# DaehwanKimLab/centrifuge

Hardware: AMD Instinct MI355X
Metric: classified reads/sec (whole node) on 100bp synthetic reads vs p_compressed; HBM GB/s achieved (higher is better)
Workload: dtype u64

## Files before the change

centrifuge_amd/csrc/cf_device.hip:

```cpp
#include <hip/hip_runtime.h>
#include <sched.h>
#include <dlfcn.h>

#include <algorithm>
#include <cmath>
#include <chrono>
#include <cstdio>
#include <cstdlib>
#include <cstring>
#include <memory>
#include <mutex>
#include <stdexcept>
#include <string>
#include <vector>

#include "../../include/centrifuge_amd.h"
#include "cf_index.hpp"
#include "cf_kernels.hpp"
#include "cf_scan.hpp"
#include "cf_textio.hpp"
#include "cf_restore.hpp"
#include "cf_plan.hpp"
#include "cf_knobs.hpp"

// ... 16 lines not shown
        if (e_ != hipSuccess)                                                                     \
            throw HipError(std::string(#expr) + ": " + hipGetErrorString(e_));                    \
    } while (0)

static thread_local uint64_t *g_dryBytes = nullptr;
template <typename T>
struct DevBuf {
    T *p = nullptr;
    size_t n = 0;
    DevBuf() = default;
    DevBuf(const DevBuf &) = delete;
    DevBuf &operator=(const DevBuf &) = delete;
    ~DevBuf() { release(); }
    void release() { if (p) (void)hipFree(p); p = nullptr; n = 0; }
    void alloc(size_t count) {
        release();
        if (count == 0) count = 1;
        if (g_dryBytes) { *g_dryBytes += count * sizeof(T); n = count; return; }
        HIP_OK(hipMalloc(reinterpret_cast<void **>(&p), count * sizeof(T)));
        n = count;
    }
    void ensure(size_t count) { if (count > n) alloc(count + count / 8); }
    void upload(const std::vector<T> &v) {
        alloc(v.size());
        if (!v.empty()) HIP_OK(hipMemcpy(p, v.data(), v.size() * sizeof(T), hipMemcpyHostToDevice));
    }
    size_t bytes() const { return n * sizeof(T); }
};

template <int G>
__global__ void __launch_bounds__(256) k_search(DIndex ix, DParams pr, DBatch b) { search_body<G>(ix, pr, b); }

__global__ void __launch_bounds__(256) k_rlen(const uint64_t *off, uint32_t *rlen, uint32_t nReads) { rlen_body(off, rlen, nReads, cf_global_thread()); }
__global__ void __launch_bounds__(256) k_convert(DConvert c) { convert_body(c, cf_global_thread()); }
__global__ void __launch_bounds__(256) k_dense_unpack(DUnpack u) { dense_unpack_body(u, (uint64_t)blockIdx.x * blockDim.x + threadIdx.x); }
__global__ void __launch_bounds__(256) k_pack(DBatch b, uint8_t *recs, uint32_t W) { pack_body(b, recs, W, cf_global_thread()); }

template <int G, int W, bool COUNT>
__global__ void __launch_bounds__(256) __attribute__((amdgpu_waves_per_eu(COUNT ? 1 : W == 4 ? 6 : W == 6 ? 5 : 4, 8))) k_search2(DIndex ix, DParams pr, DBatch b) {
    __shared__ __attribute__((aligned(16))) uint8_t lds[(256 / G) * rec_lds_stride(W) + 256 * 4 * RankTab<G>::WORDS + (256 / G) * 16 * kLazyHits];
    search2_body<G, W, COUNT>(ix, pr, b, lds);
}

template <int W, bool COUNT, int LZ = 0, bool MULTI = false>
__global__ void __launch_bounds__(256) __attribute__((amdgpu_waves_per_eu((W == 4 && LZ == 1) ? 7 : (W == 4 && MULTI) ? 6 : (W == 6 && MULTI) ? 5 : 1, 8))) k_search2_l1(DIndex ix, DParams pr, DBatch b) {
    __shared__ __attribute__((aligned(16))) uint8_t lds[256 * rec_lds_stride(W) + 256 * 16 * (LZ ? LZ : (int)lazy_hits(1, W))];
    search2_body<1, W, COUNT, true, LZ, MULTI>(ix, pr, b, lds);
}
__global__ void __launch_bounds__(256) k_pair_planes(DIndex ix, uint8_t *planes2, uint64_t nGroups) {
    pair_planes_body(ix, planes2, (uint64_t)blockIdx.x * blockDim.x + threadIdx.x, nGroups);
}
__global__ void __launch_bounds__(256) k_occ_planes(DIndex ix, uint8_t *planes, uint64_t nSides) {
    occ_planes_body(ix, planes, (uint64_t)blockIdx.x * blockDim.x + threadIdx.x, nSides);
}
__global__ void __launch_bounds__(256) k_repeat_probe(DIndex ix, uint32_t nSamples, uint32_t depth, uint32_t *hits) {
    const uint32_t i = cf_global_thread();
    bool yes = false;
    if (i < nSamples && ix.len > 2) {
        uint64_t x = 0x9e3779b97f4a7c15ull * (i + 1);
        x ^= x >> 29; x *= 0xbf58476d1ce4e5b9ull; x ^= x >> 32;
        yes = repeat_probe_body(ix, x % (ix.len - 1), depth);
    }
    const uint64_t m = cf_ballot(yes);
    if (m && cf_lane() == (uint32_t)cf_ctz64(m)) (void)cf_atomic_add(hits, (uint32_t)cf_popc64(m));
}

__global__ void __launch_bounds__(256) k_post_fast(DIndex ix, DParams pr, DBatch b) {
    const uint32_t q = cf_global_thread();
    const bool d = q < b.nQueries ? post_fast_body(ix, pr, b, q) : false;
    if (q < b.nQueries && b.postDeferred) b.postDeferred[q] = d ? 1 : 0;
    defer_push(b.slowPost, &b.st->nSlowPost, d, q);
}
template <bool EARLY>
__global__ void __launch_bounds__(256) k_score_fast(DIndex ix, DParams pr, DBatch b) {
    const uint32_t q = cf_global_thread();
    const bool d = q < b.nQueries ? score_fast_body<EARLY>(ix, pr, b, q) : false;
    defer_push(b.slowScore, &b.st->nSlowScore, d, q);
}
__global__ void __launch_bounds__(256) k_list_all(uint32_t *list, uint32_t *counter, uint32_t n) {
    const uint32_t q = cf_global_thread();
    if (q < n) list[q] = q;
    if (q == 0) *counter = n;
}
__global__ void __launch_bounds__(64) __attribute__((amdgpu_waves_per_eu(3, 8))) k_post(DIndex ix, DParams pr, DBatch b, uint32_t capHits) {
    extern __shared__ __attribute__((aligned(16))) uint8_t ldsPost[];
    HitP *scratch = capHits ? reinterpret_cast<HitP *>(ldsPost) + (size_t)cf_local_thread() * capHits : nullptr;
    const uint32_t n = b.st->nSlowPost;
    for (uint32_t i = cf_global_thread(); i < n; i += cf_global_threads()) post_body(ix, pr, b, b.slowPost[i], scratch, capHits);
}
__global__ void __launch_bounds__(64) k_postfix_only(DIndex ix, DParams pr, DBatch b) {
    const uint32_t i = cf_global_thread();
    if (i < b.st->nItems / 2) post_fix(ix, pr, b, b.items[i]);
}
__global__ void k_window(DBatch b, uint32_t qLo, bool keepSlow) { if (cf_global_thread() == 0) row_window_body(b, qLo, keepSlow); }
__global__ void __launch_bounds__(256) k_emit(DParams pr, DBatch b) {
    const uint32_t q = cf_global_thread();
    if (q < b.nQueries) emit_body(pr, b, q);
}
template <int G, bool COUNT>
__global__ void __launch_bounds__(256) k_walk2(DIndex ix, DBatch b) { walk2_body<G, COUNT>(ix, b); }
template <int MODE>
__global__ void __launch_bounds__(256) k_walk_table(DIndex ix, DBatch b) { walk2_body<2, false, MODE>(ix, b); }
template <typename T>
__global__ void __launch_bounds__(256) k_stop_samples(DIndex ix, T *stopVal, uint64_t *stopBits, uint64_t nSamples) {
    for (uint64_t i = (uint64_t)blockIdx.x * blockDim.x + threadIdx.x; i < nSamples; i += (uint64_t)gridDim.x * blockDim.x) {
        const uint64_t pos = trio_at(ix.saPos, i << ix.offRate);
        stopVal[pos] = static_cast<const T *>(ix.offs)[i];
        cf_atomic_or64(&stopBits[pos >> 6], 1ull << (pos & 63));
    }
}
template <typename T>
__global__ void __launch_bounds__(256) k_stop_bounds(DIndex ix, T *stopVal, uint64_t *stopBits) {
    for (uint64_t j = (uint64_t)blockIdx.x * blockDim.x + threadIdx.x; j < ix.nBound; j += (uint64_t)gridDim.x * blockDim.x) {
        const uint64_t pos = trio_at(ix.saPos, ix.boundRow[j]);
        stopVal[pos] = (T)ix.boundRef[j];
        cf_atomic_or64(&stopBits[pos >> 6], 1ull << (pos & 63));
    }
}
template <typename T>
__global__ void k_stop_end(DIndex ix, T *stopVal, uint64_t *stopBits) {
    const uint64_t pos = trio_at(ix.saPos, ix.zOff);
    stopVal[pos] = 0;
    cf_atomic_or64(&stopBits[pos >> 6], 1ull << (pos & 63));
}
template <typename T>
__global__ void __launch_bounds__(256) k_table_by_position(DIndex ix, const T *stopVal, const uint64_t *stopBits, T *table, uint64_t nRows, uint32_t *walkMax) {
    uint32_t gap = 0;
    for (uint64_t row = (uint64_t)blockIdx.x * blockDim.x + threadIdx.x; row < nRows; row += (uint64_t)gridDim.x * blockDim.x) {
        const uint64_t pos = trio_at(ix.saPos, row);
        uint64_t w = pos >> 6;
        uint64_t m = stopBits[w] & (~0ull >> (63 - (pos & 63)));
        while (m == 0 && w > 0) m = stopBits[--w];
        const uint64_t pred = m ? (w << 6) + 63 - (uint64_t)__builtin_clzll(m) : 0;
        table[row] = stopVal[pred];
        const uint32_t g = (uint32_t)(pos - pred);
        gap = g > gap ? g : gap;
    }
    for (int d = 32; d > 0; d >>= 1) { const uint32_t o = __shfl_xor(gap, d, 64); gap = o > gap ? o : gap; }
    if ((threadIdx.x & 63) == 0 && gap) atomicMax(walkMax, gap);
}
template <typename T>
__global__ void __launch_bounds__(256) k_table_spot_check(DIndex ix, const T *table, uint64_t nRows, uint32_t nCheck, uint32_t *bad) {
    const uint32_t i = blockIdx.x * blockDim.x + threadIdx.x;
    if (i >= nCheck) return;
    const uint64_t row = i < 64 ? (i < 32 ? (uint64_t)i : nRows - 1 - (i - 32)) % nRows : (0x9e3779b97f4a7c15ull * (i + 1)) % nRows;
    uint32_t steps = 0;
    const uint32_t want = resolve_plain_row(ix, row, steps);
    if ((uint32_t)table[row] != (sizeof(T) == 2 ? (want & 0xffffu) : want)) atomicAdd(bad, 1u);
}

template <bool COUNT>
__global__ void __launch_bounds__(256) k_walk3(DIndex ix, DBatch b) {
    for (uint64_t i = (uint64_t)blockIdx.x * blockDim.x + threadIdx.x; i < b.st->rowHi - b.st->rowLo; i += (uint64_t)gridDim.x * blockDim.x)
        walk3_body<COUNT>(ix, b, i);
}
template <bool PLANES>
__global__ void __launch_bounds__(256) k_wide_ftab(DIndex ix, uint32_t wideChars, uint64_t *table) {
    __builtin_assume(PLANES ? ix.planes != nullptr : ix.planes == nullptr);
    for (uint64_t t = (uint64_t)blockIdx.x * blockDim.x + threadIdx.x; t < (1ull << (2 * wideChars)); t += (uint64_t)gridDim.x * blockDim.x)
        wide_ftab_body(ix, wideChars, table, t);
}

__global__ void __launch_bounds__(64) k_resolve_slow(DIndex ix, DParams pr, DBatch b) {
    const uint32_t n = b.st->nSlowScore;
    for (uint32_t i = cf_global_thread(); i < n; i += cf_global_threads()) resolve_query_body(ix, pr, b, b.slowScore[i]);
}
__global__ void __launch_bounds__(64) k_score(DIndex ix, DParams pr, DBatch b, uint32_t capRows, uint32_t sparse, uint32_t rowsMin, uint32_t rowsMax) {
    extern __shared__ __attribute__((aligned(16))) uint8_t ldsScore[];
    const uint32_t n = b.st->nSlowScore;
    if (cf_local_thread() % sparse) return;
    const uint32_t me = cf_global_thread() / sparse, all = cf_global_threads() / sparse;
// ... 1128 lines not shown
    pl.nWords = bt->nWords;
    pl.pass = bt->pass.p; pl.hitCap = bt->hitCap.p; pl.slotOf = bt->slotOf.p;
    pl.hitBase = bt->hitBase.p; pl.items = bt->items.p; pl.st = bt->st.p;
    pl.itemMeta = bt->selfRecords ? bt->itemMeta.p : nullptr;
    pl.bases = bt->bases.p; pl.revDelta = bt->revDelta;
    pl.hitsCap = bt->hitsCapLimit ? std::min<uint64_t>(bt->hitsCapLimit, bt->hits.n) : bt->hits.n;
    DBatch &d = bt->d;
    d.bases = bt->bases.p; d.nmask = bt->nmask.p; d.rlen = bt->rlen.p; d.woff = bt->woff.p; d.seeds = bt->seeds.p;
    d.pass = bt->pass.p; d.items = bt->items.p; d.slotOf = bt->slotOf.p; d.hitBase = bt->hitBase.p; d.hitCap = bt->hitCap.p;
    d.lazyHits = (uint32_t)(envInt("CF_LAZY_HITS", 1) != 0) | (cl->ix->d.posFrag ? 4u : 0u);
    d.directRefs = (uint32_t)(cl->ix->dense.p && cl->ix->d.walkRate == 0 && envInt("CF_SCORE_FAST", 1) != 0 && envInt("CF_DIRECT_REFS", 1) != 0);
    d.hits = bt->hits.p; d.nhml = bt->nhml.p; d.qflag = bt->qflag.p; d.qhead = bt->qhead.p; d.qplan = bt->qplan.p; d.qplanStride = bt->qplan.n / kInlinePlan; d.qRows = bt->qRows.p; d.qBase = bt->qBase.p;
    d.rowVal = bt->rowVal.p; d.rowRef = bt->rowRef.p; d.hm = bt->hm.p; d.tc = bt->tc.p;
    d.out = bt->out.p; d.nOut = bt->nOut.p; d.score2 = bt->score2.p;
    d.counts = cl->counts.p; d.nTaxa = (uint32_t)cl->ix->h.taxa.size();
    d.nReads = (uint32_t)bt->nReads; d.nQueries = (uint32_t)bt->nQueries; d.paired = bt->paired;
    d.cursor = bt->cursor.p; d.st = bt->st.p; d.ops = bt->ops.p;
    d.slowPost = bt->slowPost.p; d.slowScore = bt->slowScore.p; d.postDeferred = envInt("CF_EARLY_SCORE", 0) ? bt->postDeferred.p : nullptr;
    d.o1tax = bt->o1tax.p; d.o1a = bt->o1a.p; d.o1b = bt->o1b.p; d.oStride = bt->o1tax.n / kFieldRows;
    d.hitsCap = pl.hitsCap;
    d.rowsCap = bt->rowsCapLimit ? std::min<uint64_t>(bt->rowsCapLimit, bt->rowVal.n) : bt->rowVal.n;
    d.recs = bt->recWords && !bt->selfRecords ? bt->recs.p : nullptr; d.recWords = bt->recWords;
    d.itemMeta = bt->selfRecords ? bt->itemMeta.p : nullptr;
}

static void enqueuePlan(cf_batch *bt, hipStream_t st) {
    const uint64_t nReads = bt->nReads;
    const DPlan &pl = bt->pl;
    HIP_OK(hipStreamWaitEvent(st, bt->ev[8], 0));
    if (bt->densePending) {
        const uint32_t L = bt->densePending - 1;
        const DUnpack u{bt->dense.p, bt->bases.p, bt->rlen.p, (uint32_t)nReads, L, bt->revDelta ? bt->bases.p + bt->revDelta : nullptr};
        bt->revMade = bt->revDelta != 0;
        const uint64_t threads = nReads * std::max<uint64_t>(((uint64_t)L + 31) >> 5, 1);
        hipLaunchKernelGGL(k_dense_unpack, dim3((unsigned)((threads + 255) / 256)), dim3(256), 0, st, u);
        bt->densePending = 0;
    }
    HIP_OK(hipEventRecord(bt->ev[5], st));
    HIP_OK(hipMemsetAsync(bt->st.p, 0, sizeof(BatchStatus), st));
    const dim3 gp((unsigned)((nReads + 1 + 255) / 256)), bl(256);
    if (bt->fromBytes && nReads) hipLaunchKernelGGL(k_rlen, gp, bl, 0, st, bt->off8.p, bt->rlen.p, (uint32_t)nReads);
    scan_enqueue<SCAN_WORDS>(bt->rlen.p, nReads, bt->woff.p, nullptr, bt->tileA.p, bt->tileC.p, st);
    if (bt->fromBytes && nReads) {
        DConvert c{bt->seq.p, bt->off8.p, bt->woff.p, bt->bases.p, bt->nmask.p, (uint32_t)nReads};
        hipLaunchKernelGGL(k_convert, dim3((unsigned)((nReads + 255) / 256)), dim3(256), 0, st, c);
    }
    if (bt->fromText && nReads) {
        const DTextPack c{bt->text.p, bt->txSeqOff.p, bt->rlen.p, bt->woff.p, bt->bases.p, bt->nmask.p, (uint32_t)nReads};
        hipLaunchKernelGGL(k_text_pack, dim3((unsigned)((nReads + 255) / 256)), dim3(256), 0, st, c);
    }
    hipLaunchKernelGGL(k_plan, gp, bl, 0, st, pl);
    scan_enqueue<SCAN_HITS>(bt->hitCap.p, nReads, bt->hitBase.p, bt->slotOf.p, bt->tileA.p, bt->tileC.p, st);
    hipLaunchKernelGGL(k_plan_fill, gp, bl, 0, st, pl);
    if (pl.revDelta && nReads && !bt->revMade) {
        const uint64_t threads = nReads * (uint64_t)bt->recWords;
        hipLaunchKernelGGL(k_rev_words, dim3((unsigned)((threads + 255) / 256)), bl, 0, st, pl, bt->recWords);
    }
    if (bt->nQueries) hipLaunchKernelGGL(k_plan_maxscore, dim3((unsigned)((bt->nQueries + 255) / 256)), bl, 0, st, bt->rlen.p, bt->pass.p,
                                         (uint32_t)bt->nQueries, bt->paired, bt->maxScore.p);
    if (bt->recWords && !bt->selfRecords && nReads) {
        const uint64_t threads = 2 * nReads * (uint64_t)bt->recWords;
        hipLaunchKernelGGL(k_pack, dim3((unsigned)((threads + 255) / 256)), bl, 0, st, bt->d, bt->recs.p, bt->recWords);
    }
    HIP_OK(hipEventRecord(bt->ev[6], st));
    bt->planned = true;
}

static dim3 listGrid(const cf_index &ix, uint64_t nq) { return dim3((unsigned)std::max<uint64_t>(1, std::min<uint64_t>((nq + 63) / 64, (uint64_t)ix.numCUs * 32))); }

static bool earlyScoreMode(const cf_batch *bt) {
    static const bool on = envInt("CF_EARLY_SCORE", 0) != 0 && envInt("CF_POST_FAST", 1) != 0 && envInt("CF_SCORE_FAST", 1) != 0 && envInt("CF_TAIL_STREAM", 0) == 0;
    return on && bt->d.directRefs != 0 && bt->tail != nullptr && bt->nQueries != 0;
}

static void enqueuePost(cf_batch *bt, hipStream_t st) {
    cf_classifier *cl = bt->cl;
    cf_index &ix = *cl->ix;
    const DBatch &d = bt->d;
    const uint32_t nq = (uint32_t)bt->nQueries;
    if (!nq) return;
    static const bool fast = envInt("CF_POST_FAST", 1) != 0;
    if (fast) hipLaunchKernelGGL(k_post_fast, dim3((nq + 255) / 256), dim3(256), 0, st, ix.d, cl->d, d);
    else hipLaunchKernelGGL(k_list_all, dim3((nq + 255) / 256), dim3(256), 0, st, bt->slowPost.p, &bt->st.p->nSlowPost, nq);
    if (earlyScoreMode(bt)) {
        HIP_OK(hipEventRecord(bt->evPostFast, st));
        HIP_OK(hipStreamWaitEvent(bt->tail, bt->evPostFast, 0));
        hipLaunchKernelGGL(k_post, listGrid(ix, nq), dim3(64), 0, bt->tail, ix.d, cl->d, d, 0u);
        HIP_OK(hipEventRecord(bt->evPost, bt->tail));
        hipLaunchKernelGGL(k_score_fast<true>, dim3((nq + 255) / 256), dim3(256), 0, st, ix.d, cl->d, d);
        HIP_OK(hipStreamWaitEvent(st, bt->evPost, 0));
        return;
    }
    static const bool postLds = envInt("CF_POST_LDS", 0) != 0;
    const uint32_t capHits = postLds ? (uint32_t)std::min<uint64_t>(60, 2 * ((uint64_t)bt->maxLenHost / (uint64_t)std::max(1, ix.h.g.ftabChars) + 2)) : 0u;
    hipLaunchKernelGGL(k_post, listGrid(ix, nq), dim3(64), (size_t)64 * capHits * sizeof(HitP), st, ix.d, cl->d, d, capHits);
}

static bool enqueueRowPass(cf_batch *bt, uint32_t qLo, hipStream_t st, bool marks, hipStream_t late = nullptr, bool early = false) {
    cf_classifier *cl = bt->cl;
    cf_index &ix = *cl->ix;
    const DBatch &d = bt->d;
    const uint32_t nq = (uint32_t)bt->nQueries;
    static const bool fast = envInt("CF_SCORE_FAST", 1) != 0;
    HIP_OK(hipMemsetAsync(bt->cursor.p + 1, 0, 8, st));
    hipLaunchKernelGGL(k_window, dim3(1), dim3(64), 0, st, d, qLo, early);
    const bool direct = d.directRefs != 0;
    if (nq && !direct) hipLaunchKernelGGL(k_emit, dim3((nq + 255) / 256), dim3(256), 0, st, cl->d, d);
    if (marks) HIP_OK(hipEventRecord(bt->ev[2], st));
    const bool counted = nq && !direct ? launchWalk(cl, bt, st) : true;
    if (marks) HIP_OK(hipEventRecord(bt->ev[3], st));
    if (nq) {
        if (early) {}
        else if (fast) hipLaunchKernelGGL(k_score_fast<false>, dim3((nq + 255) / 256), dim3(256), 0, st, ix.d, cl->d, d);
        else hipLaunchKernelGGL(k_list_all, dim3((nq + 255) / 256), dim3(256), 0, st, bt->slowScore.p, &bt->st.p->nSlowScore, nq);
        if (late && late != st) {
            HIP_OK(hipEventRecord(bt->evLate, st));
            HIP_OK(hipStreamWaitEvent(late, bt->evLate, 0));
            st = late;
        }
        if (direct) hipLaunchKernelGGL(k_resolve_slow, listGrid(ix, nq), dim3(64), 0, st, ix.d, cl->d, d);
        static const uint32_t capRows = (uint32_t)std::clamp(envInt("CF_SCORE_LDS_ROWS", 0), 0, 64), sparse = (uint32_t)std::clamp(envInt("CF_SCORE_LDS_SPARSE", 2), 1, 64);
        hipLaunchKernelGGL(k_score, listGrid(ix, nq), dim3(64), (size_t)(64 / sparse) * score_scratch_bytes(capRows), st, ix.d, cl->d, d, capRows, capRows ? sparse : 1u, 0u, 0xffffffffu);
        static const uint32_t slotBits = (uint32_t)std::clamp(envInt("CF_COUNT_SLOT_BITS", (int)kCountSlotBits), 1, (int)kCountSlotBits);
        hipLaunchKernelGGL(k_count, dim3((nq + kCountChunk - 1) / kCountChunk), dim3(1024), 0, st, d, slotBits, d.nTaxa <= (1u << slotBits));
    }
    if (marks) HIP_OK(hipEventRecord(bt->ev[4], st));
    return counted;
}

static void enqueueCompact(cf_batch *bt, hipStream_t st) {
    const uint32_t nq = (uint32_t)bt->nQueries;
    const dim3 g((nq + 1 + 255) / 256), bl(256);
    scan_enqueue<SCAN_PLAIN>(bt->nOut.p, nq, bt->rowFirst.p, nullptr, bt->tileA.p, bt->tileC.p, st);
    const bool narrow = bt->resultFormat == CF_RESULTS_NARROW;
    const DCompact c{bt->out.p, bt->o1tax.p, bt->o1a.p, bt->o1b.p, bt->d.oStride, bt->nOut.p, bt->rowFirst.p, (uint32_t)bt->cl->d.k, nq, bt->outCompact.p, bt->st.p,
                     narrow ? reinterpret_cast<NarrowRow *>(bt->outCompact.p) : nullptr, bt->qinfo.p, bt->pass.p, bt->paired};
    hipLaunchKernelGGL(k_compact, g, bl, 0, st, c);
}

static void enqueueClassify(cf_batch *bt, hipStream_t st) {
    cf_classifier *cl = bt->cl;
    HIP_OK(hipMemsetAsync(bt->cursor.p, 0, 32, st));
    HIP_OK(hipMemsetAsync(bt->ops.p, 0, sizeof(OpCounts), st));
    static const bool allFast = envInt("CF_POST_FAST", 1) != 0 && envInt("CF_SCORE_FAST", 1) != 0;
    if (!allFast) {
        HIP_OK(hipMemsetAsync(bt->qRows.p, 0, 4 * (bt->nQueries + 1), st));
        HIP_OK(hipMemsetAsync(bt->nOut.p, 0, 4 * (bt->nQueries + 1), st));
    }
    HIP_OK(hipMemsetAsync(&bt->st.p->nSlowPost, 0, 8, st));
    HIP_OK(hipEventRecord(bt->ev[0], st));
    bool counted = true;
    if (bt->nReads) counted = launchSearch(cl, bt, st) && counted;
    HIP_OK(hipEventRecord(bt->ev[1], st));
    static const int tailMode = envInt("CF_TAIL_STREAM", 0);
    hipStream_t ts = bt->tail && tailMode == 1 ? bt->tail : st;
    hipStream_t late = bt->tail && tailMode == 2 ? bt->tail : ts;
    if (ts != st) HIP_OK(hipStreamWaitEvent(ts, bt->ev[1], 0));
    const bool early = earlyScoreMode(bt);
    enqueuePost(bt, ts);
    scan_enqueue<SCAN_PLAIN>(bt->qRows.p, bt->nQueries, bt->qBase.p, nullptr, bt->tileA.p, bt->tileC.p, ts);
    counted = enqueueRowPass(bt, 0, ts, true, late, early) && counted;
    enqueueCompact(bt, late);
    HIP_OK(hipEventRecord(bt->ev[9], late));
    bt->opsValid = counted;
    bt->passes = 1;
    bt->running = true; bt->finished = false; bt->downloaded = false;
    bt->stream = st;
}

static void enqueueDownload(cf_batch *bt, hipStream_t st) {
    const uint64_t nq = bt->nQueries;
    HIP_OK(hipStreamWaitEvent(st, bt->ev[9], 0));
    HIP_OK(hipMemcpyAsync(bt->hSt.p, bt->st.p, sizeof(BatchStatus), hipMemcpyDeviceToHost, st));
    HIP_OK(hipMemcpyAsync(bt->hOps.p, bt->ops.p, sizeof(OpCounts), hipMemcpyDeviceToHost, st));
    if (nq && !bt->rowsStay) {
        const uint64_t spec = std::min<uint64_t>(bt->rowsSpec, nq * (uint64_t)bt->cl->d.k);
        if (bt->resultFormat == CF_RESULTS_NARROW) {
            HIP_OK(hipMemcpyAsync(bt->hQInfo.p, bt->qinfo.p, nq, hipMemcpyDeviceToHost, st));
// ... 1025 lines not shown
```

centrifuge_amd/csrc/cf_kernels.hpp:

```cpp
#pragma once
#include "cf_platform.hpp"

namespace cfamd {

constexpr uint32_t kNone32 = 0xffffffffu;
constexpr uint64_t kNone64 = ~0ull;
constexpr uint32_t kSideChars = 384;
constexpr int kSearchChunk = CF_WAVE;

struct RefInfo { uint64_t tax; uint32_t tidx, pid; };
static_assert(sizeof(RefInfo) == 16, "RefInfo layout");
struct DIndex {
    const uint8_t *sides;
    const uint64_t *ftab, *eftab;
    uint64_t fchr0, fchr1, fchr2, fchr3;
    uint64_t len, zOff, zSide;
    uint32_t zIn;
    int32_t ftabChars, offRate, offw;
    const void *offs;
    const uint8_t *planes;
    const uint8_t *planes2;
    const uint64_t *wide;
    int32_t wideChars;
    const uint64_t *text;
// ... 1654 lines not shown
            if (M >= 4 && M >= q - pe) {
                dep = dep + M - (uint32_t)(q - pe);
                top = trio_at(ix.isa, q >> ix.isaRate); bot = top + 1;
                continue;
            }
        }
        const int c = strand_char(b, wbase, L, fw, L - dep - 1, win);
        if (c > 3) break;
        uint64_t t, bb;
        { bool two; rank_any<G>(ix, c, top, bot, t, bb, two); }
        if (bb <= t) break;
        run = (bb - t == 1 && bot - top == 1) ? run + 1 : 0;
        top = t; bot = bb; dep++;
    }
    h.top = top; h.bot = bot; h.len = dep - cur;
}

CF_DEV bool hit_less(const HitP &a, const HitP &b) {
    const uint64_t as = hp_size(a), bs = hp_size(b);
    const uint64_t al = hp_len(a), bl = hp_len(b);
    if (al >= 22 || bl >= 22) {
        if (al >= 22 && bl >= 22) { if (as < bs) return true; if (as > bs) return false; }
        if (bl < al) return true;
        if (bl > al) return false;
    }
    if (bl * as < al * bs) return true;
    if (bl * as > al * bs) return false;
    if (as < bs) return true;
    if (as > bs) return false;
    if (bl < al) return true;
    return false;
}
CF_DEV void hit_swap(HitP &a, HitP &b) { const HitP t = a; a = b; b = t; }

CF_DEV void ss_linear_insert(HitP *a, int last) {
    const HitP val = a[last];
    int next = last - 1;
    while (hit_less(val, a[next])) { a[last] = a[next]; last = next; --next; }
    a[last] = val;
}
CF_DEV void ss_insertion(HitP *a, int first, int last) {
    if (first == last) return;
    for (int i = first + 1; i != last; ++i) {
        if (hit_less(a[i], a[first])) {
            const HitP val = a[i];
            for (int k = i; k > first; --k) a[k] = a[k - 1];
            a[first] = val;
        } else ss_linear_insert(a, i);
    }
}
CF_DEV void ss_push_heap(HitP *a, int first, int hole, int top, const HitP &val) {
    int parent = (hole - 1) / 2;
    while (hole > top && hit_less(a[first + parent], val)) {
        a[first + hole] = a[first + parent]; hole = parent; parent = (hole - 1) / 2;
    }
    a[first + hole] = val;
}
CF_DEV void ss_adjust_heap(HitP *a, int first, int hole, int len, const HitP &val) {
    const int top = hole;
    int child = hole;
    while (child < (len - 1) / 2) {
        child = 2 * (child + 1);
        if (hit_less(a[first + child], a[first + (child - 1)])) child--;
        a[first + hole] = a[first + child]; hole = child;
    }
    if ((len & 1) == 0 && child == (len - 2) / 2) {
        child = 2 * (child + 1);
        a[first + hole] = a[first + (child - 1)]; hole = child - 1;
    }
    ss_push_heap(a, first, hole, top, val);
}
CF_DEV void ss_heapsort(HitP *a, int first, int last) {
    const int len = last - first;
    if (len >= 2) {
        int parent = (len - 2) / 2;
        for (;;) { const HitP v = a[first + parent]; ss_adjust_heap(a, first, parent, len, v); if (parent == 0) break; parent--; }
    }
    while (last - first > 1) {
        --last;
        const HitP v = a[last]; a[last] = a[first];
        ss_adjust_heap(a, first, 0, last - first, v);
    }
}
CF_DEV void std_sort_hits(HitP *a, int n) {
    if (n <= 1) return;
    int lg = 0;
    for (int t = n; t > 1; t >>= 1) lg++;
    int stF[48], stL[48], stD[48], sp = 0;
    int first = 0, last = n, depth = 2 * lg;
    for (;;) {
        while (last - first > 16) {
            if (depth == 0) { ss_heapsort(a, first, last); break; }
            --depth;
            const int mid = first + (last - first) / 2;
            {
                const int x = first + 1, y = mid, z = last - 1;
                if (hit_less(a[x], a[y])) {
                    if (hit_less(a[y], a[z])) hit_swap(a[first], a[y]);
                    else if (hit_less(a[x], a[z])) hit_swap(a[first], a[z]);
                    else hit_swap(a[first], a[x]);
                } else if (hit_less(a[x], a[z])) hit_swap(a[first], a[x]);
                else if (hit_less(a[y], a[z])) hit_swap(a[first], a[z]);
                else hit_swap(a[first], a[y]);
            }
            int lo = first + 1, hi = last;
            for (;;) {
                while (hit_less(a[lo], a[first])) ++lo;
                --hi;
                while (hit_less(a[first], a[hi])) --hi;
                if (!(lo < hi)) break;
                hit_swap(a[lo], a[hi]);
                ++lo;
            }
            if (sp < 48) { stF[sp] = lo; stL[sp] = last; stD[sp] = depth; sp++; }
            last = lo;
        }
        if (sp == 0) break;
        --sp; first = stF[sp]; last = stL[sp]; depth = stD[sp];
    }
    if (n > 16) {
        ss_insertion(a, 0, 16);
        for (int i = 16; i != n; ++i) ss_linear_insert(a, i);
    } else ss_insertion(a, 0, n);
}

CF_DEV void hit_reset(HitP &h) { Hit z; z.top = z.bot = 0; z.bwoff = kNone32; z.len = 0; z.nelt = 0; h = hit_pack(z); }

CF_DEV void post_trim(HitP *h, uint32_t n) {
    if (n < 2) return;
    for (uint32_t i = 0; i + 1 < n; i++) {
        for (uint32_t j = i + 1; j < n; j++) {
            const uint32_t bi = hp_bwoff(h[i]), bj = hp_bwoff(h[j]), li = hp_len(h[i]), lj = hp_len(h[j]);
            if (bi >= bj) { hp_set_len(h[i], 0); break; }
            if ((uint64_t)bi + li <= bj) break;
            if (li >= lj) {
                const uint32_t e = bj + lj;
                hp_set_bwoff(h[j], bi + li); hp_set_len(h[j], e - (bi + li));
            } else hp_set_len(h[i], bj - bi);
        }
    }
}

CF_DEV void post_fix(const DIndex &ix, const DParams &pr, const DBatch &b, uint32_t rd, HitP *const hs[2], const uint32_t n[2]) {
    const uint64_t wbase = b.woff[rd], m = pr.m;
    const uint32_t L = b.rlen[rd];
    uint64_t sum[2] = {0, 0};
    for (int f = 0; f < 2; f++) for (uint32_t i = 0; i < n[f]; i++) if (hp_len(hs[f][i]) >= m) sum[f] += hp_len(hs[f][i]);
    if (sum[0] >= m && sum[1] >= m) {
        for (uint32_t i = 0; i < n[0]; i++) {
            HitP &hit = hs[0][i];
            const uint64_t len = hp_len(hit), l = hp_bwoff(hit), r = l + len;
            for (uint32_t j = 0; j < n[1]; j++) {
                HitP &rc = hs[1][j];
                const uint64_t rclen = hp_len(rc);
                if (len < m && rclen < m) continue;
                const uint64_t rc_l = (uint64_t)L - hp_bwoff(rc) - rclen, rc_r = rc_l + rclen;
                if (r <= rc_l) continue;
                if (rc_r <= l) continue;
                if (l == rc_l && r == rc_r) continue;
                if (l < rc_l && r > rc_r) continue;
                if (l > rc_l && r < rc_r) continue;
                if (l > rc_l) {
                    Hit t; ps_whole<1>(ix, b, wbase, L, true, (uint32_t)rc_l, t);
                    if (t.len == len + l - rc_l) hit = hit_pack(t);
                }
                if (r > rc_r) {
                    Hit t; ps_whole<1>(ix, b, wbase, L, false, (uint32_t)(L - r), t);
                    if (t.len == rclen + r - rc_r) rc = hit_pack(t);
                }
            }
        }
        for (uint32_t i = 0; i < n[0]; i++) {
            HitP &hit = hs[0][i];
            const uint64_t len = hp_len(hit), l = hp_bwoff(hit), r = l + len;
            for (uint32_t j = 0; j < n[1]; j++) {
                HitP &rc = hs[1][j];
                const uint64_t rclen = hp_len(rc), rc_l = (uint64_t)L - hp_bwoff(rc) - rclen, rc_r = rc_l + rclen;
                if (rc_l < l) break;
                if (len != rclen) continue;
                if (l == rc_l && r == rc_r && hp_size(hit) + hp_size(rc) > pr.ihits) {
                    hit_reset(hit); hit_reset(rc); break;
                }
            }
        }
    }
    post_trim(hs[0], n[0]);
    post_trim(hs[1], n[1]);
}
CF_DEV void post_fix(const DIndex &ix, const DParams &pr, const DBatch &b, uint32_t rd) {
    const uint32_t slot = b.slotOf[rd];
    HitP *hs[2] = {b.hits + b.hitBase[rd], b.hits + b.hitBase[rd] + b.hitCap[rd]};
    const uint32_t n[2] = {nhml_n(b.nhml[2 * slot]), nhml_n(b.nhml[2 * slot + 1])};
    post_fix(ix, pr, b, rd, hs, n);
}

CF_DEV void hits_copy(HitP *dst, const HitP *src, uint32_t n) {
    uint32_t i = 0;
    for (; i + 4 <= n; i += 4) { const HitP a = src[i], b2 = src[i + 1], c = src[i + 2], d = src[i + 3]; dst[i] = a; dst[i + 1] = b2; dst[i + 2] = c; dst[i + 3] = d; }
    for (; i < n; i++) dst[i] = src[i];
}

CF_DEV void post_body(const DIndex &ix, const DParams &pr, const DBatch &b, uint32_t q, HitP *scratch = nullptr, uint32_t scratchCap = 0) {
    if (b.st->flags & kStHitsOverflow) { b.qRows[q] = 0; return; }
    QHead qi;
    for (int a = 0; a < 2; a++) { qi.lo[a] = qi.hi[a] = 0; qi.nProc[a][0] = qi.nProc[a][1] = 0; qi.brk[a] = 0; qi.pad2[a] = 0; qi.maxG[a][0] = qi.maxG[a][1] = 0; }
    uint32_t nPlanned = 0;
    const uint32_t r0 = b.paired ? 2 * q : q;
    const bool p0 = b.pass[r0] != 0, p1 = b.paired ? b.pass[r0 + 1] != 0 : false;
    uint32_t rds[2] = {r0, r0 + 1};
    int nm;
    uint32_t isPaired = 0, firstMate = 0;
    if (b.paired && p0 && p1) { nm = 2; isPaired = 1; }
    else if (p0) nm = 1;
    else if (p1) { nm = 1; rds[0] = r0 + 1; firstMate = 1; }
    else nm = 0;
    const uint64_t k = pr.k, m = pr.m;
    uint64_t maxG = k;
    uint32_t rowsTotal = 0;
    uint32_t tsBase = 0;
    bool tsWide = false;
    for (int rdi = 0; rdi < nm; rdi++) {
        const uint32_t rd = rds[rdi], slot = b.slotOf[rd];
        HitP *const pool[2] = {b.hits + b.hitBase[rd], b.hits + b.hitBase[rd] + b.hitCap[rd]};
        HitP *hs[2] = {pool[0], pool[1]};
        const uint32_t hm0 = b.nhml[2 * slot], hm1 = b.nhml[2 * slot + 1];
        const uint32_t n[2] = {nhml_n(hm0), nhml_n(hm1)};
        const bool long0 = nhml_long(hm0), long1 = nhml_long(hm1);
        if (!long0 && !long1) continue;
        const uint32_t need = (long0 ? n[0] : 0u) + (long1 ? n[1] : 0u);
        const bool staged = scratch != nullptr && need <= scratchCap;
        if (staged) {
            hs[0] = scratch; hs[1] = scratch + (long0 ? n[0] : 0u);
            if (long0) hits_copy(hs[0], pool[0], n[0]);
            if (long1) hits_copy(hs[1], pool[1], n[1]);
        }
        if (long0 && long1) post_fix(ix, pr, b, rd, hs, n);
        else post_trim(hs[long0 ? 0 : 1], n[long0 ? 0 : 1]);
        uint64_t tot[2] = {0, 0}, mx[2] = {0, 0};
        for (int f = 0; f < 2; f++) if (f == 0 ? long0 : long1) for (uint32_t i = 0; i < n[f]; i++) {
            const uint64_t len = hp_len(hs[f][i]);
            if (len < m) continue;
            tot[f] += (len - 15) * (len - 15);
            if (len > mx[f]) mx[f] = len;
        }
        int lo, hi;
        if (tot[0] != tot[1]) { lo = tot[0] > tot[1] ? 0 : 1; hi = lo + 1; }
        else if (mx[0] != mx[1]) { lo = mx[0] > mx[1] ? 0 : 1; hi = lo + 1; }
        else { lo = 0; hi = 2; }
        qi.lo[rdi] = (uint8_t)lo; qi.hi[rdi] = (uint8_t)hi;
        for (int f = lo; f < hi; f++) {
            HitP *h = hs[f];
            for (uint32_t i = 0; i < n[f]; i++)
                if (hp_len(h[i]) >= m && hp_size(h[i]) > maxG) maxG = hp_size(h[i]);
            if (maxG > k) maxG += k;
            qi.maxG[rdi][f] = maxG > 0xffffffffull ? 0xffffffffu : (uint32_t)maxG;
            std_sort_hits(h, (int)n[f]);
            uint64_t cnt = 0;
            uint32_t i = 0;
            for (; i < n[f]; i++) {
                const uint64_t len = hp_len(h[i]), size = hp_size(h[i]);
                const uint64_t nelt = plan_nelt(len, size, maxG, m, pr.ihits);
                if (nelt == 0) continue;
                if (nPlanned < kInlinePlan) {
                    PlanHit ph;
                    ph.top = hp_row(h[i]); ph.nelt = (uint32_t)nelt; ph.meta = plan_meta((uint32_t)len, rdi, f, tsBase + i);
                    if (tsBase + i > kPlanTsMax || len > 0xffffu) tsWide = true;
                    b.qplan[(uint64_t)nPlanned * b.qplanStride + q] = ph;
                }
                nPlanned++;
                rowsTotal += (uint32_t)nelt;
                cnt += nelt;
                if (cnt >= maxG) { i++; qi.brk[rdi] |= (uint8_t)(1u << f); break; }
            }
            qi.nProc[rdi][f] = i;
            tsBase += i - ((qi.brk[rdi] >> f) & 1u);
            if (staged) hits_copy(pool[f], h, n[f]);
        }
    }
    const uint32_t nPlan = (nPlanned <= kInlinePlan && !tsWide) ? nPlanned : kPlanNotInline;
    b.qflag[q] = qf_make(nPlan, isPaired, firstMate, (uint32_t)nm);
    if (nPlan == kPlanNotInline) b.qhead[q] = qi;
    b.qRows[q] = rowsTotal;
}

CF_DEV void defer_push(uint32_t *list, uint32_t *counter, bool defer, uint32_t q) {
    const uint64_t mask = cf_ballot(defer);
    if (!mask) return;
    const uint32_t lane = cf_lane();
    const int leader = cf_ctz64(mask);
    uint32_t base = 0;
    if ((int)lane == leader) base = cf_atomic_add(counter, (uint32_t)cf_popc64(mask));
    base = cf_shfl(base, leader);
    if (defer) list[base + (uint32_t)cf_popc64(mask & ((1ull << lane) - 1))] = q;
}

constexpr int kPostFastHits = 8;
CF_DEV bool post_fast_body(const DIndex &ix, const DParams &pr, const DBatch &b, uint32_t q) {
    (void)ix;
    if (b.st->flags & kStHitsOverflow) { b.qRows[q] = 0; return false; }
    uint32_t fOf0 = 2, fOf1 = 2, np0 = 0, np1 = 0, brk0 = 0, brk1 = 0;
    uint8_t isPaired = 0, firstMate = 0;
    const uint32_t r0 = b.paired ? 2 * q : q;
    const bool p0 = b.pass[r0] != 0, p1 = b.paired ? b.pass[r0 + 1] != 0 : false;
    uint32_t rd0 = r0;
    int nm;
    if (b.paired && p0 && p1) { nm = 2; isPaired = 1; }
    else if (p0) nm = 1;
    else if (p1) { nm = 1; rd0 = r0 + 1; firstMate = 1; }
    else nm = 0;
    const uint64_t k = pr.k, m = pr.m;
    uint64_t maxG = k;
    uint32_t rowsTotal = 0, tsBase = 0, nPlanned = 0;
    PlanHit pl0{0, 0, 0}, pl1{0, 0, 0}, pl2{0, 0, 0}, pl3{0, 0, 0};
    static_assert(kInlinePlan == 4, "four plan slots below");
    bool defer = false;
    for (int rdi = 0; rdi < nm && !defer; rdi++) {
        const uint32_t rd = rd0 + (uint32_t)rdi, slot = b.slotOf[rd];
        const uint32_t hm0 = b.nhml[2 * slot], hm1 = b.nhml[2 * slot + 1];
        const bool long0 = nhml_long(hm0), long1 = nhml_long(hm1);
        if (!long0 && !long1) continue;
        if (long0 && long1) { defer = true; break; }
        const int f = long0 ? 0 : 1;
        const uint32_t n = nhml_n(f ? hm1 : hm0);
        if (n > (uint32_t)kPostFastHits) { defer = true; break; }
        const uint8_t *hp = reinterpret_cast<const uint8_t *>(b.hits + b.hitBase[rd] + (f ? b.hitCap[rd] : 0u));
        uint64_t w0[kPostFastHits], w1[kPostFastHits];
#pragma unroll
        for (int i = 0; i < kPostFastHits; i++) {
            u64x2 v{0, 0};
            if ((uint32_t)i < n) v = cf_load16(hp + 16 * i);
            w0[i] = v.x; w1[i] = v.y;
        }
        bool apart = true;
        uint64_t mg = maxG;
#pragma unroll
        for (int i = 0; i < kPostFastHits; i++) {
            if ((uint32_t)i >= n) continue;
            const HitP hi{w0[i], w1[i]};
            const uint64_t len = hp_len(hi), size = hp_size(hi);
            if (len >= m && size > mg) mg = size;
            if (i + 1 < kPostFastHits && (uint32_t)(i + 1) < n) {
                const HitP hj{w0[i + 1], w1[i + 1]};
                const uint64_t bi = hp_bwoff(hi), bj = hp_bwoff(hj);
                if (bi >= bj || bi + len > bj) apart = false;
            }
        }
        if (!apart) { defer = true; break; }
        maxG = mg;
        if (maxG > k) maxG += k;
        uint32_t rank[kPostFastHits];
#pragma unroll
        for (int i = 0; i < kPostFastHits; i++) rank[i] = 0;
#pragma unroll
        for (int i = 0; i < kPostFastHits; i++) {
#pragma unroll
            for (int j = i + 1; j < kPostFastHits; j++) {
                if ((uint32_t)j < n) {
                    const bool jFirst = hit_less(HitP{w0[j], w1[j]}, HitP{w0[i], w1[i]});
                    rank[i] += jFirst ? 1u : 0u;
                    rank[j] += jFirst ? 0u : 1u;
                }
            }
        }
        uint64_t cnt = 0;
        uint32_t visited = n;
// ... 850 lines not shown
```

Before: 1.427 billion.

## Cooperative post-processing: lane groups precompute post_fix extension searches into LDS memo

Restructures the slow post kernel so a group of G lanes (default 4) handles one query. The leader gathers the distinct post_fix re-search candidates into an LDS key list, the group runs the ps_whole searches in parallel and memoizes them, and the leader then runs the serial fix, sort and plan logic against the memo. The sort stack and QHead move into LDS with a packed 64-bit stack entry, which cuts per-thread register and scratch pressure. In exchange most lanes sit idle during the serial leader phases, the optional per-thread LDS staging path is removed, and the grid is now sized per wave.

Result: faster. 1.459 billion, median of 6 (+2.2%).

```diff
diff --git a/centrifuge_amd/csrc/cf_device.hip b/centrifuge_amd/csrc/cf_device.hip
--- a/centrifuge_amd/csrc/cf_device.hip
+++ b/centrifuge_amd/csrc/cf_device.hip
@@ -122,11 +122,10 @@
     if (q < n) list[q] = q;
     if (q == 0) *counter = n;
 }
-__global__ void __launch_bounds__(64) __attribute__((amdgpu_waves_per_eu(3, 8))) k_post(DIndex ix, DParams pr, DBatch b, uint32_t capHits) {
-    extern __shared__ __attribute__((aligned(16))) uint8_t ldsPost[];
-    HitP *scratch = capHits ? reinterpret_cast<HitP *>(ldsPost) + (size_t)cf_local_thread() * capHits : nullptr;
-    const uint32_t n = b.st->nSlowPost;
-    for (uint32_t i = cf_global_thread(); i < n; i += cf_global_threads()) post_body(ix, pr, b, b.slowPost[i], scratch, capHits);
+template <int G>
+__global__ void __launch_bounds__(64) __attribute__((amdgpu_waves_per_eu(3, 8))) k_post(DIndex ix, DParams pr, DBatch b) {
+    __shared__ __attribute__((aligned(16))) PostGroupLds ldsPost[64 / G];
+    post_wave_body<G>(ix, pr, b, ldsPost);
 }
 __global__ void __launch_bounds__(64) k_postfix_only(DIndex ix, DParams pr, DBatch b) {
     const uint32_t i = cf_global_thread();
@@ -1421,18 +1420,29 @@
     static const bool fast = envInt("CF_POST_FAST", 1) != 0;
     if (fast) hipLaunchKernelGGL(k_post_fast, dim3((nq + 255) / 256), dim3(256), 0, st, ix.d, cl->d, d);
     else hipLaunchKernelGGL(k_list_all, dim3((nq + 255) / 256), dim3(256), 0, st, bt->slowPost.p, &bt->st.p->nSlowPost, nq);
+    static const int group = envInt("CF_POST_GROUP", 4);
+    const auto launchPost = [&](hipStream_t s) {
+        const auto go = [&](auto kern, uint32_t perWave) {
+            const dim3 grid((unsigned)std::max<uint64_t>(1, std::min<uint64_t>(((uint64_t)nq + perWave - 1) / perWave, (uint64_t)ix.numCUs * 32)));
+            hipLaunchKernelGGL(kern, grid, dim3(64), 0, s, ix.d, cl->d, d);
+        };
+        switch (group) {
+            case 8: go(k_post<8>, 8); break;
+            case 16: go(k_post<16>, 4); break;
+            case 64: go(k_post<64>, 1); break;
+            default: go(k_post<4>, 16); break;
+        }
+    };
     if (earlyScoreMode(bt)) {
         HIP_OK(hipEventRecord(bt->evPostFast, st));
         HIP_OK(hipStreamWaitEvent(bt->tail, bt->evPostFast, 0));
-        hipLaunchKernelGGL(k_post, listGrid(ix, nq), dim3(64), 0, bt->tail, ix.d, cl->d, d, 0u);
+        launchPost(bt->tail);
         HIP_OK(hipEventRecord(bt->evPost, bt->tail));
         hipLaunchKernelGGL(k_score_fast<true>, dim3((nq + 255) / 256), dim3(256), 0, st, ix.d, cl->d, d);
         HIP_OK(hipStreamWaitEvent(st, bt->evPost, 0));
         return;
     }
-    static const bool postLds = envInt("CF_POST_LDS", 0) != 0;
-    const uint32_t capHits = postLds ? (uint32_t)std::min<uint64_t>(60, 2 * ((uint64_t)bt->maxLenHost / (uint64_t)std::max(1, ix.h.g.ftabChars) + 2)) : 0u;
-    hipLaunchKernelGGL(k_post, listGrid(ix, nq), dim3(64), (size_t)64 * capHits * sizeof(HitP), st, ix.d, cl->d, d, capHits);
+    launchPost(st);
 }
 
 static bool enqueueRowPass(cf_batch *bt, uint32_t qLo, hipStream_t st, bool marks, hipStream_t late = nullptr, bool early = false) {
diff --git a/centrifuge_amd/csrc/cf_kernels.hpp b/centrifuge_amd/csrc/cf_kernels.hpp
--- a/centrifuge_amd/csrc/cf_kernels.hpp
+++ b/centrifuge_amd/csrc/cf_kernels.hpp
@@ -1760,11 +1760,12 @@
         ss_adjust_heap(a, first, 0, last - first, v);
     }
 }
-CF_DEV void std_sort_hits(HitP *a, int n) {
+constexpr int kSortStack = 48;
+CF_DEV void std_sort_hits(HitP *a, int n, uint64_t *stk) {
     if (n <= 1) return;
     int lg = 0;
     for (int t = n; t > 1; t >>= 1) lg++;
-    int stF[48], stL[48], stD[48], sp = 0;
+    int sp = 0;
     int first = 0, last = n, depth = 2 * lg;
     for (;;) {
         while (last - first > 16) {
@@ -1790,17 +1791,18 @@
                 hit_swap(a[lo], a[hi]);
                 ++lo;
             }
-            if (sp < 48) { stF[sp] = lo; stL[sp] = last; stD[sp] = depth; sp++; }
+            if (sp < kSortStack) stk[sp++] = (uint64_t)lo | ((uint64_t)last << 28) | ((uint64_t)depth << 56);
             last = lo;
         }
         if (sp == 0) break;
-        --sp; first = stF[sp]; last = stL[sp]; depth = stD[sp];
+        --sp; first = (int)(stk[sp] & 0xfffffffu); last = (int)((stk[sp] >> 28) & 0xfffffffu); depth = (int)(stk[sp] >> 56);
     }
     if (n > 16) {
         ss_insertion(a, 0, 16);
         for (int i = 16; i != n; ++i) ss_linear_insert(a, i);
     } else ss_insertion(a, 0, n);
 }
+CF_DEV void std_sort_hits(HitP *a, int n) { uint64_t stk[kSortStack]; std_sort_hits(a, n, stk); }
 
 CF_DEV void hit_reset(HitP &h) { Hit z; z.top = z.bot = 0; z.bwoff = kNone32; z.len = 0; z.nelt = 0; h = hit_pack(z); }
 
@@ -1819,9 +1821,9 @@
     }
 }
 
-CF_DEV void post_fix(const DIndex &ix, const DParams &pr, const DBatch &b, uint32_t rd, HitP *const hs[2], const uint32_t n[2]) {
-    const uint64_t wbase = b.woff[rd], m = pr.m;
-    const uint32_t L = b.rlen[rd];
+template <typename PS>
+CF_DEV void post_fix_with(const DParams &pr, uint32_t L, HitP *const hs[2], const uint32_t n[2], PS &&ps) {
+    const uint64_t m = pr.m;
     uint64_t sum[2] = {0, 0};
     for (int f = 0; f < 2; f++) for (uint32_t i = 0; i < n[f]; i++) if (hp_len(hs[f][i]) >= m) sum[f] += hp_len(hs[f][i]);
     if (sum[0] >= m && sum[1] >= m) {
@@ -1839,12 +1841,12 @@
                 if (l < rc_l && r > rc_r) continue;
                 if (l > rc_l && r < rc_r) continue;
                 if (l > rc_l) {
-                    Hit t; ps_whole<1>(ix, b, wbase, L, true, (uint32_t)rc_l, t);
-                    if (t.len == len + l - rc_l) hit = hit_pack(t);
+                    const HitP t = ps(true, (uint32_t)rc_l);
+                    if (hp_len(t) == len + l - rc_l) hit = t;
                 }
                 if (r > rc_r) {
-                    Hit t; ps_whole<1>(ix, b, wbase, L, false, (uint32_t)(L - r), t);
-                    if (t.len == rclen + r - rc_r) rc = hit_pack(t);
+                    const HitP t = ps(false, (uint32_t)(L - r));
+                    if (hp_len(t) == rclen + r - rc_r) rc = t;
                 }
             }
         }
@@ -1865,6 +1867,32 @@
     post_trim(hs[0], n[0]);
     post_trim(hs[1], n[1]);
 }
+template <typename ADD>
+CF_DEV void post_fix_candidates(const DParams &pr, uint32_t L, const HitP *const hs[2], const uint32_t n[2], ADD &&add) {
+    const uint64_t m = pr.m;
+    uint64_t sum[2] = {0, 0};
+    for (int f = 0; f < 2; f++) for (uint32_t i = 0; i < n[f]; i++) if (hp_len(hs[f][i]) >= m) sum[f] += hp_len(hs[f][i]);
+    if (sum[0] < m || sum[1] < m) return;
+    for (uint32_t i = 0; i < n[0]; i++) {
+        const uint64_t len = hp_len(hs[0][i]), l = hp_bwoff(hs[0][i]), r = l + len;
+        for (uint32_t j = 0; j < n[1]; j++) {
+            const uint64_t rclen = hp_len(hs[1][j]);
+            if (len < m && rclen < m) continue;
+            const uint64_t rc_l = (uint64_t)L - hp_bwoff(hs[1][j]) - rclen, rc_r = rc_l + rclen;
+            if (r <= rc_l || rc_r <= l) continue;
+            if (l == rc_l && r == rc_r) continue;
+            if (l < rc_l && r > rc_r) continue;
+            if (l > rc_l && r < rc_r) continue;
+            if (l > rc_l) add(true, (uint32_t)rc_l);
+            if (r > rc_r) add(false, (uint32_t)(L - r));
+        }
+    }
+}
+CF_DEV void post_fix(const DIndex &ix, const DParams &pr, const DBatch &b, uint32_t rd, HitP *const hs[2], const uint32_t n[2]) {
+    const uint64_t wbase = b.woff[rd];
+    const uint32_t L = b.rlen[rd];
+    post_fix_with(pr, L, hs, n, [&](bool fw, uint32_t cur) { Hit t; ps_whole<1>(ix, b, wbase, L, fw, cur, t); return hit_pack(t); });
+}
 CF_DEV void post_fix(const DIndex &ix, const DParams &pr, const DBatch &b, uint32_t rd) {
     const uint32_t slot = b.slotOf[rd];
     HitP *hs[2] = {b.hits + b.hitBase[rd], b.hits + b.hitBase[rd] + b.hitCap[rd]};
@@ -1878,27 +1906,88 @@
     for (; i < n; i++) dst[i] = src[i];
 }
 
+struct PostAcc {
+    uint64_t maxG;
+    uint32_t nPlanned, rowsTotal;
+    uint32_t tsBase;
+    bool tsWide;
+};
+CF_DEV int post_mates(const DBatch &b, uint32_t q, uint32_t &rd0, uint32_t &isPaired, uint32_t &firstMate) {
+    const uint32_t r0 = b.paired ? 2 * q : q;
+    const bool p0 = b.pass[r0] != 0, p1 = b.paired ? b.pass[r0 + 1] != 0 : false;
+    rd0 = r0; isPaired = 0; firstMate = 0;
+    if (b.paired && p0 && p1) { isPaired = 1; return 2; }
+    if (p0) return 1;
+    if (p1) { rd0 = r0 + 1; firstMate = 1; return 1; }
+    return 0;
+}
+CF_DEV void qhead_clear(QHead &qi) {
+    for (int a = 0; a < 2; a++) { qi.lo[a] = qi.hi[a] = 0; qi.nProc[a][0] = qi.nProc[a][1] = 0; qi.brk[a] = 0; qi.pad2[a] = 0; qi.maxG[a][0] = qi.maxG[a][1] = 0; }
+}
+CF_DEV void post_plan_mate(const DParams &pr, const DBatch &b, uint32_t q, int rdi, HitP *const hs[2], HitP *const pool[2], const uint32_t n[2],
+                           bool long0, bool long1, bool staged, QHead &qi, PostAcc &acc, uint64_t *sortStk) {
+    const uint64_t k = pr.k, m = pr.m;
+    uint64_t tot[2] = {0, 0}, mx[2] = {0, 0};
+    for (int f = 0; f < 2; f++) if (f == 0 ? long0 : long1) for (uint32_t i = 0; i < n[f]; i++) {
+        const uint64_t len = hp_len(hs[f][i]);
+        if (len < m) continue;
+        tot[f] += (len - 15) * (len - 15);
+        if (len > mx[f]) mx[f] = len;
+    }
+    int lo, hi;
+    if (tot[0] != tot[1]) { lo = tot[0] > tot[1] ? 0 : 1; hi = lo + 1; }
+    else if (mx[0] != mx[1]) { lo = mx[0] > mx[1] ? 0 : 1; hi = lo + 1; }
+    else { lo = 0; hi = 2; }
+    qi.lo[rdi] = (uint8_t)lo; qi.hi[rdi] = (uint8_t)hi;
+    uint64_t maxG = acc.maxG;
+    for (int f = lo; f < hi; f++) {
+        HitP *h = f == 0 ? hs[0] : hs[1];
+        const uint32_t nf = f == 0 ? n[0] : n[1];
+        for (uint32_t i = 0; i < nf; i++)
+            if (hp_len(h[i]) >= m && hp_size(h[i]) > maxG) maxG = hp_size(h[i]);
+        if (maxG > k) maxG += k;
+        qi.maxG[rdi][f] = maxG > 0xffffffffull ? 0xffffffffu : (uint32_t)maxG;
+        std_sort_hits(h, (int)nf, sortStk);
+        uint64_t cnt = 0;
+        uint32_t i = 0;
+        for (; i < nf; i++) {
+            const uint64_t len = hp_len(h[i]), size = hp_size(h[i]);
+            const uint64_t nelt = plan_nelt(len, size, maxG, m, pr.ihits);
+            if (nelt == 0) continue;
+            if (acc.nPlanned < kInlinePlan) {
+                PlanHit ph;
+                ph.top = hp_row(h[i]); ph.nelt = (uint32_t)nelt; ph.meta = plan_meta((uint32_t)len, rdi, f, acc.tsBase + i);
+                if (acc.tsBase + i > kPlanTsMax || len > 0xffffu) acc.tsWide = true;
+                b.qplan[(uint64_t)acc.nPlanned * b.qplanStride + q] = ph;
+            }
+            acc.nPlanned++;
+            acc.rowsTotal += (uint32_t)nelt;
+            cnt += nelt;
+            if (cnt >= maxG) { i++; qi.brk[rdi] |= (uint8_t)(1u << f); break; }
+        }
+        qi.nProc[rdi][f] = i;
+        acc.tsBase += i - ((qi.brk[rdi] >> f) & 1u);
+        if (staged) hits_copy(f == 0 ? pool[0] : pool[1], h, nf);
+    }
+    acc.maxG = maxG;
+}
+CF_DEV void post_finish(const DBatch &b, uint32_t q, const QHead &qi, const PostAcc &acc, uint32_t isPaired, uint32_t firstMate, int nm) {
+    const uint32_t nPlan = (acc.nPlanned <= kInlinePlan && !acc.tsWide) ? acc.nPlanned : kPlanNotInline;
+    b.qflag[q] = qf_make(nPlan, isPaired, firstMate, (uint32_t)nm);
+    if (nPlan == kPlanNotInline) b.qhead[q] = qi;
+    b.qRows[q] = acc.rowsTotal;
+}
+
 CF_DEV void post_body(const DIndex &ix, const DParams &pr, const DBatch &b, uint32_t q, HitP *scratch = nullptr, uint32_t scratchCap = 0) {
     if (b.st->flags & kStHitsOverflow) { b.qRows[q] = 0; return; }
     QHead qi;
-    for (int a = 0; a < 2; a++) { qi.lo[a] = qi.hi[a] = 0; qi.nProc[a][0] = qi.nProc[a][1] = 0; qi.brk[a] = 0; qi.pad2[a] = 0; qi.maxG[a][0] = qi.maxG[a][1] = 0; }
-    uint32_t nPlanned = 0;
-    const uint32_t r0 = b.paired ? 2 * q : q;
-    const bool p0 = b.pass[r0] != 0, p1 = b.paired ? b.pass[r0 + 1] != 0 : false;
-    uint32_t rds[2] = {r0, r0 + 1};
-    int nm;
-    uint32_t isPaired = 0, firstMate = 0;
-    if (b.paired && p0 && p1) { nm = 2; isPaired = 1; }
-    else if (p0) nm = 1;
-    else if (p1) { nm = 1; rds[0] = r0 + 1; firstMate = 1; }
-    else nm = 0;
-    const uint64_t k = pr.k, m = pr.m;
-    uint64_t maxG = k;
-    uint32_t rowsTotal = 0;
-    uint32_t tsBase = 0;
-    bool tsWide = false;
+    qhead_clear(qi);
+    PostAcc acc{pr.k, 0, 0, 0, false};
+    uint32_t rd0, isPaired, firstMate;
+    const int nm = post_mates(b, q, rd0, isPaired, firstMate);
+    uint64_t sortStk[kSortStack];
     for (int rdi = 0; rdi < nm; rdi++) {
-        const uint32_t rd = rds[rdi], slot = b.slotOf[rd];
+        const uint32_t rd = rd0 + (uint32_t)rdi, slot = b.slotOf[rd];
         HitP *const pool[2] = {b.hits + b.hitBase[rd], b.hits + b.hitBase[rd] + b.hitCap[rd]};
         HitP *hs[2] = {pool[0], pool[1]};
         const uint32_t hm0 = b.nhml[2 * slot], hm1 = b.nhml[2 * slot + 1];
@@ -1914,51 +2003,85 @@
         }
         if (long0 && long1) post_fix(ix, pr, b, rd, hs, n);
         else post_trim(hs[long0 ? 0 : 1], n[long0 ? 0 : 1]);
-        uint64_t tot[2] = {0, 0}, mx[2] = {0, 0};
-        for (int f = 0; f < 2; f++) if (f == 0 ? long0 : long1) for (uint32_t i = 0; i < n[f]; i++) {
-            const uint64_t len = hp_len(hs[f][i]);
-            if (len < m) continue;
-            tot[f] += (len - 15) * (len - 15);
-            if (len > mx[f]) mx[f] = len;
-        }
-        int lo, hi;
-        if (tot[0] != tot[1]) { lo = tot[0] > tot[1] ? 0 : 1; hi = lo + 1; }
-        else if (mx[0] != mx[1]) { lo = mx[0] > mx[1] ? 0 : 1; hi = lo + 1; }
-        else { lo = 0; hi = 2; }
-        qi.lo[rdi] = (uint8_t)lo; qi.hi[rdi] = (uint8_t)hi;
-        for (int f = lo; f < hi; f++) {
-            HitP *h = hs[f];
-            for (uint32_t i = 0; i < n[f]; i++)
-                if (hp_len(h[i]) >= m && hp_size(h[i]) > maxG) maxG = hp_size(h[i]);
-            if (maxG > k) maxG += k;
-            qi.maxG[rdi][f] = maxG > 0xffffffffull ? 0xffffffffu : (uint32_t)maxG;
-            std_sort_hits(h, (int)n[f]);
-            uint64_t cnt = 0;
-            uint32_t i = 0;
-            for (; i < n[f]; i++) {
-                const uint64_t len = hp_len(h[i]), size = hp_size(h[i]);
-                const uint64_t nelt = plan_nelt(len, size, maxG, m, pr.ihits);
-                if (nelt == 0) continue;
-                if (nPlanned < kInlinePlan) {
-                    PlanHit ph;
-                    ph.top = hp_row(h[i]); ph.nelt = (uint32_t)nelt; ph.meta = plan_meta((uint32_t)len, rdi, f, tsBase + i);
-                    if (tsBase + i > kPlanTsMax || len > 0xffffu) tsWide = true;
-                    b.qplan[(uint64_t)nPlanned * b.qplanStride + q] = ph;
-                }
-                nPlanned++;
-                rowsTotal += (uint32_t)nelt;
-                cnt += nelt;
-                if (cnt >= maxG) { i++; qi.brk[rdi] |= (uint8_t)(1u << f); break; }
-            }
-            qi.nProc[rdi][f] = i;
-            tsBase += i - ((qi.brk[rdi] >> f) & 1u);
-            if (staged) hits_copy(pool[f], h, n[f]);
-        }
-    }
-    const uint32_t nPlan = (nPlanned <= kInlinePlan && !tsWide) ? nPlanned : kPlanNotInline;
-    b.qflag[q] = qf_make(nPlan, isPaired, firstMate, (uint32_t)nm);
-    if (nPlan == kPlanNotInline) b.qhead[q] = qi;
-    b.qRows[q] = rowsTotal;
+        post_plan_mate(pr, b, q, rdi, hs, pool, n, long0, long1, staged, qi, acc, sortStk);
+    }
+    post_finish(b, q, qi, acc, isPaired, firstMate, nm);
+}
+
+constexpr uint32_t kPostMemo = 16;
+struct PostGroupLds {
+    HitP memo[kPostMemo];
+    uint32_t key[kPostMemo];
+    uint64_t sortStk[kSortStack];
+    QHead qi;
+    uint32_t pad[2];
+};
+static_assert(sizeof(PostGroupLds) % 16 == 0, "PostGroupLds: 16-byte records first");
+CF_DEV uint32_t post_key(bool fw, uint32_t cur) { return (fw ? 0x80000000u : 0u) | cur; }
+template <int G, uint32_t MEMO = kPostMemo>
+CF_DEV void post_wave_body(const DIndex &ix, const DParams &pr, const DBatch &b, PostGroupLds *lds) {
+    static_assert(MEMO >= 1 && MEMO <= kPostMemo, "the memo's room");
+    static_assert(G >= 1 && G <= CF_WAVE && (G & (G - 1)) == 0, "a group is a power of two of lanes within a wavefront");
+    constexpr uint32_t QPW = CF_WAVE / G;
+    const uint32_t lane = cf_lane(), sub = lane & (G - 1), leader = lane & ~(uint32_t)(G - 1);
+    PostGroupLds &my = lds[(cf_local_thread() / CF_WAVE) * QPW + lane / G];
+    const uint32_t nList = b.st->nSlowPost;
+    const bool overflow = (b.st->flags & kStHitsOverflow) != 0;
+    const uint32_t wave = cf_global_thread() / CF_WAVE, nWaves = cf_global_threads() / CF_WAVE;
+    for (uint32_t base = wave * QPW; base < nList; base += nWaves * QPW) {
+        const bool active = base + lane / G < nList;
+        const bool first = active && sub == 0;
+        const uint32_t q = active ? b.slowPost[base + lane / G] : 0;
+        if (overflow) { if (first) b.qRows[q] = 0; continue; }
+        PostAcc acc{pr.k, 0, 0, 0, false};
+        uint32_t rd0 = 0, isPaired = 0, firstMate = 0;
+        int nm = 0;
+        if (first) { nm = post_mates(b, q, rd0, isPaired, firstMate); qhead_clear(my.qi); }
+        for (int rdi = 0; rdi < 2; rdi++) {
+            uint32_t rd = 0, L = 0, nCand = 0, n[2] = {0, 0};
+            uint64_t wbase = 0;
+            HitP *hs[2] = {nullptr, nullptr};
+            bool long0 = false, long1 = false;
+            if (first && rdi < nm) {
+                rd = rd0 + (uint32_t)rdi;
+                const uint32_t slot = b.slotOf[rd];
+                const uint32_t hm0 = b.nhml[2 * slot], hm1 = b.nhml[2 * slot + 1];
+                n[0] = nhml_n(hm0); n[1] = nhml_n(hm1);
+                long0 = nhml_long(hm0); long1 = nhml_long(hm1);
+                hs[0] = b.hits + b.hitBase[rd]; hs[1] = hs[0] + b.hitCap[rd];
+                if (long0 && long1) {
+                    L = b.rlen[rd]; wbase = b.woff[rd];
+                    post_fix_candidates(pr, L, hs, n, [&](bool fw, uint32_t cur) {
+                        const uint32_t key = post_key(fw, cur);
+                        for (uint32_t c = 0; c < nCand; c++) if (my.key[c] == key) return;
+                        if (nCand < MEMO) my.key[nCand++] = key;
+                    });
+                }
+            }
+            nCand = cf_shfl(nCand, (int)leader);
+            if (cf_ballot(nCand != 0)) {
+                if (G > 1) { L = cf_shfl(L, (int)leader); wbase = cf_shfl(wbase, (int)leader); }
+                cf_compiler_fence();
+                for (uint32_t c = sub; c < nCand; c += G) {
+                    const uint32_t key = my.key[c];
+                    Hit t; ps_whole<1>(ix, b, wbase, L, (key >> 31) != 0, key & 0x7fffffffu, t);
+                    my.memo[c] = hit_pack(t);
+                }
+                cf_compiler_fence();
+            }
+            if (!(first && rdi < nm) || (!long0 && !long1)) continue;
+            if (long0 && long1) {
+                post_fix_with(pr, L, hs, n, [&](bool fw, uint32_t cur) {
+                    const uint32_t key = post_key(fw, cur);
+                    for (uint32_t c = 0; c < nCand; c++) if (my.key[c] == key) return my.memo[c];
+                    Hit t; ps_whole<1>(ix, b, wbase, L, fw, cur, t);
+                    return hit_pack(t);
+                });
+            } else post_trim(long0 ? hs[0] : hs[1], long0 ? n[0] : n[1]);
+            post_plan_mate(pr, b, q, rdi, hs, hs, n, long0, long1, false, my.qi, acc, my.sortStk);
+        }
+        if (first) post_finish(b, q, my.qi, acc, isPaired, firstMate, nm);
+    }
 }
 
 CF_DEV void defer_push(uint32_t *list, uint32_t *counter, bool defer, uint32_t q) {
```
